# rongzhao-zhang/EfficientQ

Hardware: AMD Instinct MI355X
Metric: ptq_calibration_throughput (higher is better)
Workload: dtype i8xi8->i32 (exact) for the Gram systems and per-iteration loss convs of the layers with quantised input, f32/f64 elsewhere

## Files before the change

efficientq_amd/csrc/solve.hip:

```cpp
#include <cstdlib>
#include <vector>
#include "common.h"
#include "internal.h"

namespace effq {

typedef float f32x16 __attribute__((ext_vector_type(16)));
typedef double f64x4 __attribute__((ext_vector_type(4)));
typedef float f32x4 __attribute__((ext_vector_type(4)));

static inline int round_up(int v, int m) { return (v + m - 1) / m * m; }

constexpr int NBK = 64;
constexpr int LDA_S = 66;
constexpr int LDB_S = 80;

__global__ __launch_bounds__(256) void k_build_a64(const float* __restrict__ A0, int n, int npad, int has_bias,
                                                   double rho, double eta, double* __restrict__ A64) {
  const size_t tot = (size_t)npad * npad;
  const size_t stride = (size_t)gridDim.x * blockDim.x;
  for (size_t e = (size_t)blockIdx.x * blockDim.x + threadIdx.x; e < tot; e += stride) {
    const int i = (int)(e / npad), j = (int)(e % npad);
    double v = 0.0;
    if (i < n && j < n) {
// ... 333 lines not shown
      ra[v] = *reinterpret_cast<const f64x2*>(Ag + v * 32);
      rb[v] = *reinterpret_cast<const f64x2*>(Bg + v * 32);
    }
#pragma unroll
    for (int v = 0; v < 4; ++v) {
      *reinterpret_cast<f64x2*>(&As[0][sk * BG_LD + sc + v * 32]) = ra[v];
      *reinterpret_cast<f64x2*>(&Bs[0][sk * BG_LD + sc + v * 32]) = rb[v];
    }
    lds_barrier();
    for (int c = 0; c < nch; ++c) {
      const int buf = c & 1;
      if (c + 1 < nch) {
        const size_t off = (size_t)(c + 1) * BG_KC * p.ldx;
#pragma unroll
        for (int v = 0; v < 4; ++v) {
          ra[v] = *reinterpret_cast<const f64x2*>(Ag + off + v * 32);
          rb[v] = *reinterpret_cast<const f64x2*>(Bg + off + v * 32);
        }
      }
      if (live) {
#pragma unroll
        for (int ks = 0; ks < BG_KC / 4; ++ks) {
          double a[4], b[4];
#pragma unroll
          for (int mi = 0; mi < 4; ++mi) a[mi] = As[buf][(ks * 4 + lk) * BG_LD + wr * 64 + mi * 16 + lr];
#pragma unroll
          for (int ni = 0; ni < 4; ++ni) b[ni] = Bs[buf][(ks * 4 + lk) * BG_LD + wc * 64 + ni * 16 + lr];
#pragma unroll
          for (int mi = 0; mi < 4; ++mi)
#pragma unroll
            for (int ni = 0; ni < 4; ++ni)
              acc[mi][ni] = __builtin_amdgcn_mfma_f64_16x16x4f64(a[mi], b[ni], acc[mi][ni], 0, 0, 0);
        }
      }
      if (c + 1 < nch) {
#pragma unroll
        for (int v = 0; v < 4; ++v) {
          *reinterpret_cast<f64x2*>(&As[buf ^ 1][sk * BG_LD + sc + v * 32]) = ra[v];
          *reinterpret_cast<f64x2*>(&Bs[buf ^ 1][sk * BG_LD + sc + v * 32]) = rb[v];
        }
      }
      lds_barrier();
    }
  }
  if (live) {
    double* Ob = p.Cout + ((size_t)bi * NBK - p.orow) * p.ldout + ((size_t)bj * NBK - p.ocol);
#pragma unroll
    for (int mi = 0; mi < 4; ++mi)
#pragma unroll
      for (int ni = 0; ni < 4; ++ni)
#pragma unroll
        for (int r = 0; r < 4; ++r) Ob[(size_t)(mi * 16 + lk + 4 * r) * p.ldout + ni * 16 + lr] = acc[mi][ni][r];
  }
}

__global__ __launch_bounds__(256) void k_gj_panel_w(const double* __restrict__ A, int npad, int kb0, int m,
                                                    const double* __restrict__ Dw, double* __restrict__ NZT,
                                                    double* __restrict__ XTW, size_t ldx) {
  extern __shared__ __attribute__((aligned(16))) double sm[];
  double* As = sm;
  double* Bs = sm + NBK * LDA_S;
  const int t = blockIdx.x, c = blockIdx.y;
  if (t >= kb0 && t < kb0 + m) return;
  const int tid = threadIdx.x, lane = tid & 63, wid = tid >> 6;
  const int wr = wid >> 1, wc = wid & 1;
  const bool upper = t < kb0;
  const double sgn = upper ? -1.0 : 1.0;
  const int ldd = m * NBK;
  f64x4 acc[2][2];
#pragma unroll
  for (int mi = 0; mi < 2; ++mi)
#pragma unroll
    for (int ni = 0; ni < 2; ++ni)
#pragma unroll
      for (int r = 0; r < 4; ++r) acc[mi][ni][r] = 0.0;
  for (int a = 0; a < m; ++a) {
    for (int e = tid; e < NBK * NBK; e += 256) {
      const int r = e >> 6, cc = e & 63;
      if (upper)
        As[r * LDA_S + cc] = A[(size_t)(t * NBK + r) * npad + (size_t)(kb0 + a) * NBK + cc];
      else
        As[cc * LDA_S + r] = A[(size_t)((kb0 + a) * NBK + r) * npad + (size_t)t * NBK + cc];
    }
    load_tile(Bs, LDB_S, Dw + (size_t)a * NBK * ldd + (size_t)c * NBK, (size_t)ldd);
    lds_barrier();
    if (a == c)
      for (int e = tid; e < NBK * NBK; e += 256) {
        const int kk = e >> 6, r = e & 63;
        XTW[(size_t)(c * NBK + kk) * ldx + (size_t)t * NBK + r] = sgn * As[r * LDA_S + kk];
      }
    tile_mma64(As, Bs, acc);
    lds_barrier();
  }
  const int lr = lane & 15, lk = lane >> 4;
#pragma unroll
  for (int mi = 0; mi < 2; ++mi)
#pragma unroll
    for (int ni = 0; ni < 2; ++ni)
#pragma unroll
      for (int r = 0; r < 4; ++r)
        As[(wr * 32 + mi * 16 + lk + 4 * r) * LDA_S + wc * 32 + ni * 16 + lr] = acc[mi][ni][r];
  lds_barrier();
  for (int e = tid; e < NBK * NBK; e += 256) {
    const int kk = e >> 6, r = e & 63;
    NZT[(size_t)(c * NBK + kk) * ldx + (size_t)t * NBK + r] = -As[r * LDA_S + kk];
  }
}

__global__ __launch_bounds__(256) void k_gj_wback_w(double* __restrict__ A, int npad, int kb0, int m,
                                                    const double* __restrict__ Dw, const double* __restrict__ NZT,
                                                    size_t ldx) {
  __shared__ double Ts[NBK * (NBK + 1)];
  const int t = blockIdx.x, c = blockIdx.y, tid = threadIdx.x;
  const int ldd = m * NBK;
  if (t >= kb0 && t < kb0 + m) {
    const int a = t - kb0;
    if (a > c) return;
    for (int e = tid; e < NBK * NBK; e += 256) {
      const int r = e >> 6, cc = e & 63;
      A[(size_t)(t * NBK + r) * npad + (size_t)(kb0 + c) * NBK + cc] = Dw[(size_t)(a * NBK + r) * ldd + (size_t)c * NBK + cc];
    }
    return;
  }
  if (t < kb0) {
    for (int e = tid; e < NBK * NBK; e += 256) {
      const int kk = e >> 6, r = e & 63;
      Ts[kk * (NBK + 1) + r] = NZT[(size_t)(c * NBK + kk) * ldx + (size_t)t * NBK + r];
    }
    __syncthreads();
    for (int e = tid; e < NBK * NBK; e += 256) {
      const int r = e >> 6, kk = e & 63;
      A[(size_t)(t * NBK + r) * npad + (size_t)(kb0 + c) * NBK + kk] = Ts[kk * (NBK + 1) + r];
    }
  } else {
    for (int e = tid; e < NBK * NBK; e += 256) {
      const int kk = e >> 6, r = e & 63;
      A[(size_t)((kb0 + c) * NBK + kk) * npad + (size_t)t * NBK + r] = -NZT[(size_t)(c * NBK + kk) * ldx + (size_t)t * NBK + r];
    }
  }
}

constexpr int PF_LD = 130;
__device__ __forceinline__ f64x4 mm16(f64x4 acc, const double* Aop, int a_rs, int a_cs, const double* Bop, int b_rs,
                                      int b_cs, int K, int lr, int lk) {
#pragma unroll 4
  for (int ks = 0; ks < K / 4; ++ks) {
    const double a = Aop[lr * a_rs + (ks * 4 + lk) * a_cs];
    const double b = Bop[(ks * 4 + lk) * b_rs + lr * b_cs];
    acc = __builtin_amdgcn_mfma_f64_16x16x4f64(a, b, acc, 0, 0, 0);
  }
  return acc;
}

__global__ __launch_bounds__(1024) void k_gj_pivot_fused(const double* __restrict__ A, int npad, int k0, int mk,
                                                         const double* __restrict__ NZT, const double* __restrict__ XTW,
                                                         size_t ldx, int kdim, double* __restrict__ Dw) {
  extern __shared__ __attribute__((aligned(16))) double sm[];
  double* M = sm;
  double(*fcol)[NBK + 1] = reinterpret_cast<double(*)[NBK + 1]>(sm + 2 * NBK * PF_LD);
  const int tid = threadIdx.x, lane = tid & 63, wid = tid >> 6;
  const int tr = wid >> 2, tc = wid & 3;
  const int lr = lane & 15, lk = lane >> 4;
  for (int bi = 0; bi < mk; ++bi)
    for (int bj = bi; bj < mk; ++bj) {
      const size_t row0 = (size_t)(k0 + bi) * NBK + tr * 16, col0 = (size_t)(k0 + bj) * NBK + tc * 16;
      f64x4 acc;
#pragma unroll
      for (int r = 0; r < 4; ++r) acc[r] = A[(row0 + lk + 4 * r) * npad + col0 + lr];
      const double* Ag = NZT + row0 + lr;
      const double* Bg = XTW + col0 + lr;
#pragma unroll 8
      for (int ks = 0; ks < kdim / 4; ++ks) {
        const double a = Ag[(size_t)(ks * 4 + lk) * ldx];
        const double b = Bg[(size_t)(ks * 4 + lk) * ldx];
        acc = __builtin_amdgcn_mfma_f64_16x16x4f64(a, b, acc, 0, 0, 0);
      }
#pragma unroll
      for (int r = 0; r < 4; ++r) {
        const int rr = bi * NBK + tr * 16 + lk + 4 * r, cc = bj * NBK + tc * 16 + lr;
        M[rr * PF_LD + cc] = acc[r];
        if (bi < bj) M[cc * PF_LD + rr] = acc[r];
      }
    }
  lds_barrier();
  constexpr int CPW = NBK / 16;
  auto invert64 = [&](int off) {
    double reg[CPW];
#pragma unroll
    for (int j = 0; j < CPW; ++j) reg[j] = M[(off + lane) * PF_LD + off + wid * CPW + j];
    gj_invert_regs<CPW>(reg, fcol, lane, wid);
#pragma unroll
    for (int j = 0; j < CPW; ++j) M[(off + lane) * PF_LD + off + wid * CPW + j] = reg[j];
    lds_barrier();
  };
  auto zero = []() {
    f64x4 z;
#pragma unroll
    for (int r = 0; r < 4; ++r) z[r] = 0.0;
    return z;
  };
  auto tile_store = [&](int rb, int cb, f64x4 v, double sgn) {
#pragma unroll
    for (int r = 0; r < 4; ++r) M[(rb + tr * 16 + lk + 4 * r) * PF_LD + cb + tc * 16 + lr] = sgn * v[r];
  };
  auto tile_load = [&](int rb, int cb) {
    f64x4 v;
#pragma unroll
    for (int r = 0; r < 4; ++r) v[r] = M[(rb + tr * 16 + lk + 4 * r) * PF_LD + cb + tc * 16 + lr];
    return v;
  };
  invert64(0);
  if (mk == 2) {
    f64x4 z = mm16(zero(), M + (NBK + tr * 16) * PF_LD, PF_LD, 1, M + tc * 16, PF_LD, 1, NBK, lr, lk);
    lds_barrier();
    tile_store(NBK, 0, z, 1.0);
    lds_barrier();
    f64x4 sacc = tile_load(NBK, NBK);
#pragma unroll
    for (int r = 0; r < 4; ++r) sacc[r] = -sacc[r];
    sacc = mm16(sacc, M + (NBK + tr * 16) * PF_LD, PF_LD, 1, M + NBK + tc * 16, PF_LD, 1, NBK, lr, lk);
    tile_store(NBK, NBK, sacc, -1.0);
    lds_barrier();
    invert64(NBK);
    f64x4 w = mm16(zero(), M + (NBK + tr * 16) * PF_LD + NBK, PF_LD, 1, M + NBK * PF_LD + tc * 16, PF_LD, 1, NBK, lr, lk);
    tile_store(0, NBK, w, 1.0);
    lds_barrier();
    f64x4 d = tile_load(0, 0);
    d = mm16(d, M + NBK * PF_LD + tr * 16, 1, PF_LD, M + NBK + tc * 16, PF_LD, 1, NBK, lr, lk);
    tile_store(0, 0, d, 1.0);
    lds_barrier();
  }
  const int nd = mk * NBK;
  for (int e = tid; e < nd * nd; e += 1024) {
    const int i = e / nd, j = e % nd;
    double v;
    if (i < NBK && j >= NBK)
      v = -M[(j - NBK) * PF_LD + NBK + i];
    else if (i >= NBK && j < NBK)
      v = -M[(i - NBK) * PF_LD + NBK + j];
    else
      v = M[i * PF_LD + j];
    Dw[e] = v;
  }
}

__global__ __launch_bounds__(256) void k_mirror_blocks(double* __restrict__ D, int nd) {
  const size_t tot = (size_t)nd * nd;
  for (size_t e = (size_t)blockIdx.x * blockDim.x + threadIdx.x; e < tot; e += (size_t)gridDim.x * blockDim.x) {
    const int i = (int)(e / nd), j = (int)(e % nd);
    if ((i / NBK) > (j / NBK)) D[e] = D[(size_t)j * nd + i];
  }
}

__global__ __launch_bounds__(256) void k_build_b(const float* __restrict__ B0, const float* __restrict__ W0,
                                                 const float* __restrict__ b0, const float* __restrict__ G,
                                                 const float* __restrict__ dual, int c2, int n, int has_bias,
                                                 float rho, float eta, float* __restrict__ Bm, int ldb, int c2p,
                                                 const float* __restrict__ wprev, float shift) {
  const size_t tot = (size_t)c2p * ldb;
  const size_t stride = (size_t)gridDim.x * blockDim.x;
  const int nw = n - has_bias;
  for (size_t e = (size_t)blockIdx.x * blockDim.x + threadIdx.x; e < tot; e += stride) {
    const int r = (int)(e / ldb), k = (int)(e % ldb);
    float v = 0.0f;
    if (r < c2 && k < n) {
      if (k < nw) {
        const size_t wi = (size_t)r * nw + k;
        v = B0[(size_t)r * n + k] + eta * W0[wi];
        v = v + rho * (G[wi] - dual[wi]);
        if (wprev != nullptr) v = v + shift * wprev[wi];
      } else {
        v = B0[(size_t)r * n + k] + eta * b0[r];
      }
    }
    Bm[e] = v;
  }
}

__global__ __launch_bounds__(256) void k_build_b4(const float* __restrict__ B0, const float* __restrict__ W0,
                                                  const float* __restrict__ b0, const float* __restrict__ G,
                                                  const float* __restrict__ dual, int c2, int n, int has_bias,
                                                  float rho, float eta, float* __restrict__ Bm, int ldb,
                                                  const float* __restrict__ wprev, float shift) {
  __builtin_amdgcn_s_setprio(2);

  const int r = blockIdx.y;
  const int nw = n - has_bias;
  float* out = Bm + (size_t)r * ldb;
  for (int k = (blockIdx.x * blockDim.x + threadIdx.x) * 4; k < ldb; k += gridDim.x * blockDim.x * 4) {
    float4 v = make_float4(0.f, 0.f, 0.f, 0.f);
    if (r < c2 && k < nw) {
      const size_t wi = (size_t)r * nw + k;
      const float* bp = B0 + (size_t)r * n + k;
      const float4 w0 = *reinterpret_cast<const float4*>(W0 + wi), g = *reinterpret_cast<const float4*>(G + wi),
                   du = *reinterpret_cast<const float4*>(dual + wi);
      v.x = bp[0] + eta * w0.x;
      v.y = bp[1] + eta * w0.y;
      v.z = bp[2] + eta * w0.z;
      v.w = bp[3] + eta * w0.w;
      v.x = v.x + rho * (g.x - du.x);
      v.y = v.y + rho * (g.y - du.y);
      v.z = v.z + rho * (g.z - du.z);
      v.w = v.w + rho * (g.w - du.w);
      if (wprev != nullptr) {
        const float4 wp = *reinterpret_cast<const float4*>(wprev + wi);
        v.x = v.x + shift * wp.x;
        v.y = v.y + shift * wp.y;
        v.z = v.z + shift * wp.z;
        v.w = v.w + shift * wp.w;
      }
    } else if (r < c2 && k == nw && has_bias) {
      v.x = B0[(size_t)r * n + k] + eta * b0[r];
    }
    *reinterpret_cast<float4*>(out + k) = v;
  }
}

__global__ __launch_bounds__(256) void k_prox_reduce4(const float* __restrict__ part, int ldp, int nsplit, int c2, int n,
                                                      int has_bias, float* __restrict__ wstar, float* __restrict__ bstar) {
  __builtin_amdgcn_s_setprio(2);

  const int r = blockIdx.y;
  const int nw = n - has_bias;
  const size_t tot = (size_t)c2 * ldp;
  const float* row = part + (size_t)r * ldp;
  for (int k = (blockIdx.x * blockDim.x + threadIdx.x) * 4; k < ldp; k += gridDim.x * blockDim.x * 4) {
    if (k >= n) continue;
    float4 v = *reinterpret_cast<const float4*>(row + k);
    for (int z = 1; z < nsplit; ++z) {
      const float4 t = *reinterpret_cast<const float4*>(row + (size_t)z * tot + k);
      v.x += t.x;
      v.y += t.y;
      v.z += t.z;
      v.w += t.w;
    }
    if (k < nw)
      *reinterpret_cast<float4*>(wstar + (size_t)r * nw + k) = v;
    else
      bstar[r] = v.x;
  }
}

constexpr int PBK = 32, PLD = PBK + 4;

template <int MT, int WM, int WN, int NTN>
__global__ __launch_bounds__(256) void k_prox_gemm(const float* __restrict__ Bm, int ldb, const float* __restrict__ Ainv,
                                                   int lda, int n, int c2, int has_bias, float* __restrict__ wstar,
                                                   float* __restrict__ bstar, float* __restrict__ part, int ldp) {
  __builtin_amdgcn_s_setprio(2);

  constexpr int BM = 32 * MT * WM, BN = 32 * WN * NTN;
  constexpr int NA = BM * 8 / 256, NB = BN * 8 / 256;
  static_assert(WM * WN == 4 && NA >= 1 && NB >= 1, "4 waves");
  __shared__ __attribute__((aligned(16))) float As[BM * PLD];
  __shared__ __attribute__((aligned(16))) float Bs[BN * PLD];
  const int tid = threadIdx.x, lane = tid & 63, wid = tid >> 6;
  const int li = lane & 31, lh = lane >> 5;
  const int wm = wid / WN, wn = wid % WN;
  const int row0 = blockIdx.y * BM, col0 = blockIdx.x * BN;

  f32x16 acc[MT][NTN];
#pragma unroll
  for (int m = 0; m < MT; ++m)
#pragma unroll
    for (int t = 0; t < NTN; ++t)
#pragma unroll
      for (int r = 0; r < 16; ++r) acc[m][t][r] = 0.0f;

  f32x4 ra[NA], rb[NB];
  const float* pa[NA];
  const float* pb[NB];
#pragma unroll
  for (int q = 0; q < NA; ++q) {
    const int u = tid + q * 256, r = u >> 3, c4 = u & 7;
    pa[q] = Bm + (size_t)(row0 + r) * ldb + c4 * 4;
  }
#pragma unroll
  for (int q = 0; q < NB; ++q) {
    const int u = tid + q * 256, r = u >> 3, c4 = u & 7;
    pb[q] = Ainv + (size_t)min(col0 + r, n - 1) * lda + c4 * 4;
  }
#define EFFQ_PROX_FETCH(k0)                                                         \
  {                                                                                 \
    _Pragma("unroll") for (int q = 0; q < NA; ++q)                                  \
        ra[q] = *reinterpret_cast<const f32x4*>(pa[q] + (k0));                      \
    _Pragma("unroll") for (int q = 0; q < NB; ++q)                                  \
        rb[q] = *reinterpret_cast<const f32x4*>(pb[q] + (k0));                      \
  }
  const int nkt = ldb / PBK;
  const int kt0 = (int)(((long long)nkt * blockIdx.z) / gridDim.z);
  const int nk = (int)(((long long)nkt * (blockIdx.z + 1)) / gridDim.z);
  EFFQ_PROX_FETCH(kt0 * PBK)
  for (int kt = kt0; kt < nk; ++kt) {
    lds_barrier();
#pragma unroll
    for (int q = 0; q < NA; ++q) {
      const int u = tid + q * 256;
      *reinterpret_cast<f32x4*>(&As[(u >> 3) * PLD + (u & 7) * 4]) = ra[q];
    }
#pragma unroll
    for (int q = 0; q < NB; ++q) {
      const int u = tid + q * 256;
      *reinterpret_cast<f32x4*>(&Bs[(u >> 3) * PLD + (u & 7) * 4]) = rb[q];
// ... 112 lines not shown
  }
#define EFFQ_B3_FETCH(k0)                                                           \
  {                                                                                 \
    _Pragma("unroll") for (int q = 0; q < NA; ++q)                                  \
        ra[q] = *reinterpret_cast<const f32x4*>(pa[q] + (k0));                      \
    _Pragma("unroll") for (int q = 0; q < NB; ++q)                                  \
        rb[q] = *reinterpret_cast<const f32x4*>(pb[q] + (k0));                      \
  }
#define EFFQ_B3_STORE(stage)                                                                        \
  {                                                                                                 \
    __bf16* As_ = lds + (stage) * STAGE;                                                            \
    __bf16* Bs_ = As_ + 3 * BM * B3_LD;                                                             \
    _Pragma("unroll") for (int q = 0; q < NA; ++q) {                                                \
      const int u = tid + q * 512, off = (u >> 2) * B3_LD + (u & 3) * 4;                            \
      bf16x4 p0, p1, p2;                                                                            \
      split3(ra[q], p0, p1, p2);                                                                    \
      *reinterpret_cast<bf16x4*>(&As_[off]) = p0;                                                   \
      *reinterpret_cast<bf16x4*>(&As_[BM * B3_LD + off]) = p1;                                      \
      *reinterpret_cast<bf16x4*>(&As_[2 * BM * B3_LD + off]) = p2;                                  \
    }                                                                                               \
    _Pragma("unroll") for (int q = 0; q < NB; ++q) {                                                \
      const int u = tid + q * 512, off = (u >> 2) * B3_LD + (u & 3) * 4;                            \
      bf16x4 p0, p1, p2;                                                                            \
      split3(rb[q], p0, p1, p2);                                                                    \
      *reinterpret_cast<bf16x4*>(&Bs_[off]) = p0;                                                   \
      *reinterpret_cast<bf16x4*>(&Bs_[BN * B3_LD + off]) = p1;                                      \
      *reinterpret_cast<bf16x4*>(&Bs_[2 * BN * B3_LD + off]) = p2;                                  \
    }                                                                                               \
  }
  const int nkt = ldb / B3_K;
  const int kt0 = (int)(((long long)nkt * blockIdx.z) / gridDim.z);
  const int nk = (int)(((long long)nkt * (blockIdx.z + 1)) / gridDim.z);
  EFFQ_B3_FETCH(kt0 * B3_K)
  EFFQ_B3_STORE(0)
  EFFQ_B3_FETCH(min(kt0 + 1, nk - 1) * B3_K)
  lds_barrier();
  for (int kt = kt0; kt < nk; ++kt) {
    const int st = (kt - kt0) & 1;
    if (kt + 1 < nk) EFFQ_B3_STORE(st ^ 1)
    EFFQ_B3_FETCH(min(kt + 2, nk - 1) * B3_K)
    const __bf16* As = lds + st * STAGE;
    const __bf16* Bs = As + 3 * BM * B3_LD;
    bf16x8 a[MT][3], b[NT][3];
#pragma unroll
    for (int m = 0; m < MT; ++m)
#pragma unroll
      for (int p = 0; p < 3; ++p)
        a[m][p] = *reinterpret_cast<const bf16x8*>(&As[p * BM * B3_LD + ((wm * MT + m) * 32 + li) * B3_LD + 8 * lh]);
#pragma unroll
    for (int t = 0; t < NT; ++t)
#pragma unroll
      for (int p = 0; p < 3; ++p)
        b[t][p] = *reinterpret_cast<const bf16x8*>(&Bs[p * BN * B3_LD + ((wn * NT + t) * 32 + li) * B3_LD + 8 * lh]);
#pragma unroll
    for (int m = 0; m < MT; ++m)
#pragma unroll
      for (int t = 0; t < NT; ++t) {
        acc[m][t] = __builtin_amdgcn_mfma_f32_32x32x16_bf16(a[m][0], b[t][2], acc[m][t], 0, 0, 0);
        acc[m][t] = __builtin_amdgcn_mfma_f32_32x32x16_bf16(a[m][1], b[t][1], acc[m][t], 0, 0, 0);
        acc[m][t] = __builtin_amdgcn_mfma_f32_32x32x16_bf16(a[m][2], b[t][0], acc[m][t], 0, 0, 0);
        acc[m][t] = __builtin_amdgcn_mfma_f32_32x32x16_bf16(a[m][0], b[t][1], acc[m][t], 0, 0, 0);
        acc[m][t] = __builtin_amdgcn_mfma_f32_32x32x16_bf16(a[m][1], b[t][0], acc[m][t], 0, 0, 0);
        acc[m][t] = __builtin_amdgcn_mfma_f32_32x32x16_bf16(a[m][0], b[t][0], acc[m][t], 0, 0, 0);
      }
    lds_barrier();
  }
#undef EFFQ_B3_FETCH
#undef EFFQ_B3_STORE
  const int nw = n - has_bias;
  float* P = (gridDim.z > 1) ? part + (size_t)blockIdx.z * c2 * ldp : nullptr;
#pragma unroll
  for (int m = 0; m < MT; ++m)
#pragma unroll
    for (int t = 0; t < NT; ++t) {
      const int col = col0 + (wn * NT + t) * 32 + li;
#pragma unroll
      for (int r = 0; r < 16; ++r) {
        const int row = row0 + (wm * MT + m) * 32 + (r & 3) + 8 * (r >> 2) + 4 * lh;
        if (row < c2 && col < n) {
          if (P != nullptr)
            P[(size_t)row * ldp + col] = acc[m][t][r];
          else if (col < nw)
            wstar[(size_t)row * nw + col] = acc[m][t][r];
          else
            bstar[row] = acc[m][t][r];
        }
      }
    }
}

__global__ __launch_bounds__(256) void k_prox_reduce(const float* __restrict__ part, int ldp, int nsplit, int c2, int n,
                                                     int has_bias, float* __restrict__ wstar, float* __restrict__ bstar) {
  const size_t tot = (size_t)c2 * ldp, stride = (size_t)gridDim.x * blockDim.x;
  const int nw = n - has_bias;
  for (size_t e = (size_t)blockIdx.x * blockDim.x + threadIdx.x; e < tot; e += stride) {
    const int row = (int)(e / ldp), col = (int)(e % ldp);
    if (col >= n) continue;
    float v = part[e];
    for (int z = 1; z < nsplit; ++z) v += part[(size_t)z * tot + e];
    if (col < nw)
      wstar[(size_t)row * nw + col] = v;
    else
      bstar[row] = v;
  }
}

struct ProxPlan { int variant, gx, gy, nsplit, c2p, ldb; };
static ProxPlan prox_plan(int c2, int n) {
  ProxPlan p;
  p.c2p = (c2 > 128) ? round_up(c2, 256) : (c2 > 64) ? 128 : round_up(c2, 32);
  p.ldb = round_up(n, 32);
  if (p.c2p >= 128 && n >= 1024) {
    p.variant = 5; p.gx = (n + 255) / 256; p.gy = p.c2p / 256;
    if (p.c2p == 128) { p.variant = 7; p.gx = (n + 127) / 128; p.gy = 1; }
    const int tiles5 = p.gx * p.gy, nkt5 = p.ldb / B3_K;
    int s5 = (256 + tiles5 / 2) / tiles5;
    if (s5 > nkt5 / 16) s5 = nkt5 / 16;
    if (s5 < 1) s5 = 1;
    p.nsplit = s5;
    return p;
  }
  if (p.c2p >= 256) { p.variant = 0; p.gx = (n + 63) / 64; p.gy = p.c2p / 256; }
  else if (p.c2p == 128) { p.variant = 1; p.gx = (n + 63) / 64; p.gy = 1; }
  else if (p.c2p == 64) { p.variant = 2; p.gx = (n + 63) / 64; p.gy = 1; }
  else { p.variant = 3; p.gx = (n + 127) / 128; p.gy = 1; }
  const int tiles = p.gx * p.gy, nkt = p.ldb / PBK;
  int s = (440 + tiles - 1) / tiles;
  if (s > nkt / 6) s = nkt / 6;
  if (s > 16) s = 16;
  if (s < 1) s = 1;
  if (p.variant == 0) {
    const int smax = s > 1 ? 16 : 1;
    double best = -1.0;
    for (int c = 1; c <= smax && c <= nkt / 6; ++c) {
      const int wgs = tiles * c, rounds = (wgs + 767) / 768;
      const double score = (double)wgs / (768.0 * rounds) - 0.01 * c;
      if (score > best) { best = score; s = c; }
    }
  }
  p.nsplit = s;
  return p;
}

}

using namespace effq;

extern "C" {

static size_t gj64_aux_doubles(size_t npad) { return 2 * (size_t)NBK * npad + 2 * NBK * NBK; }

constexpr int GJ_WIDE_MIN_BLOCKS = 100;
static bool gj_takes_wide(int nblk) { return nblk >= GJ_WIDE_MIN_BLOCKS; }
static int gj_wide_pivot(int nblk) { return (nblk >= 100) ? effq::WB : 2; }

size_t effq_spd_inverse_ws_bytes(int n) {
  if (n <= 0) return 0;
  const size_t npad = (size_t)round_up(n, NBK);
  size_t d = npad * npad + gj64_aux_doubles(npad);
  if (gj_takes_wide((int)(npad / NBK))) {
    const size_t ldx = (size_t)round_up((int)npad, BG_T);
    d = npad * npad + 2 * (size_t)WK * ldx + (size_t)WK * WK + gj64_aux_doubles(WK);
  }
  return d * sizeof(double) + 256;
}

int effq_ainv_ld(int n) { return n > 0 ? round_up(n, 32) : 0; }

static int gj64_sweep(double* A64, int npad, double* aux, hipStream_t st) {
  const int nblk = npad / NBK;
  double* XT = aux;
  double* NZ = XT + (size_t)NBK * npad;
  double* Dinv = NZ + (size_t)NBK * npad;
  const size_t lds = (size_t)(NBK * LDA_S + NBK * LDB_S) * sizeof(double);
  for (int k = 0; k < nblk; ++k) {
    const int kb = k * NBK;
    double* Dk = Dinv + (size_t)(k & 1) * NBK * NBK;
    double* Dn = Dinv + (size_t)((k + 1) & 1) * NBK * NBK;
    if (k == 0) hipLaunchKernelGGL(k_gj_diag, dim3(1), dim3(GJD_T), 0, st, A64, npad, kb, Dk);
    hipLaunchKernelGGL(k_gj_panel, dim3(nblk), dim3(256), lds, st, A64, npad, kb, Dk, NZ, XT);
    if (nblk > 1)
      hipLaunchKernelGGL(k_gj_trail_sym, dim3((nblk + GJ_CT - 1) / GJ_CT, nblk + 1), dim3(256), 0, st, A64, npad, kb, NZ,
                         XT, Dn);
    EFFQ_LAUNCH_CHECK();
  }
  return EFFQ_OK;
}

struct GjWideCtx {
  int dev;
  hipStream_t caller, helper;
  hipEvent_t e1, e2;
};
static thread_local std::vector<GjWideCtx> g_gj_ctx;

static int gj_wide_ctx(hipStream_t caller, GjWideCtx** out) {
  int dev = 0;
  EFFQ_HIP(hipGetDevice(&dev));
  for (GjWideCtx& c : g_gj_ctx)
    if (c.dev == dev && c.caller == caller) {
      *out = &c;
      return EFFQ_OK;
    }
  GjWideCtx c;
  c.dev = dev;
  c.caller = caller;
  int prio = 0;
  if (hipStreamGetPriority(caller, &prio) != hipSuccess) prio = 0;
  EFFQ_HIP(hipStreamCreateWithPriority(&c.helper, hipStreamNonBlocking, prio));
  EFFQ_HIP(hipEventCreateWithFlags(&c.e1, hipEventDisableTiming));
  EFFQ_HIP(hipEventCreateWithFlags(&c.e2, hipEventDisableTiming));
  g_gj_ctx.push_back(c);
  *out = &g_gj_ctx.back();
  return EFFQ_OK;
}

static int gj_wide_sweep(double* A64, int npad, double* aux, hipStream_t st) {
  const int nblk = npad / NBK;
  const int WB = gj_wide_pivot(nblk);
  const size_t ldx = (size_t)round_up(npad, BG_T);
  double* NZT = aux;
  double* XTW = NZT + (size_t)WK * ldx;
  double* Dw = XTW + (size_t)WK * ldx;
  double* aux64 = Dw + (size_t)WK * WK;
  const int nK = (nblk + WB - 1) / WB, nm = (nblk + 1) / 2;
  GjWideCtx* ctx = nullptr;
  if (nK > 1) {
    const int rc = gj_wide_ctx(st, &ctx);
    if (rc != EFFQ_OK) return rc;
  }
  hipStream_t s2 = ctx ? ctx->helper : st;
  const size_t lds = (size_t)(NBK * LDA_S + NBK * LDB_S) * sizeof(double);
  const size_t pf_lds = (size_t)(2 * NBK * PF_LD + 2 * (NBK + 1)) * sizeof(double);
  auto pivot_block = [&](int k0, int mk, int kdim, hipStream_t s) -> int {
    GjBig g;
    memset(&g, 0, sizeof(g));
    g.Cin = A64; g.ldin = (size_t)npad;
    g.Cout = Dw; g.ldout = (size_t)mk * NBK; g.orow = k0 * NBK; g.ocol = k0 * NBK;
    g.NZT = NZT; g.XTW = XTW; g.ldx = ldx; g.kdim = kdim; g.nblk = nblk;
    g.i0m = k0 / 2; g.j0m = k0 / 2;
    g.skip_lo = g.skip_hi = -1; g.la_lo = g.la_hi = -1;
    if (WB == 2) {
      hipLaunchKernelGGL(k_gj_pivot_fused, dim3(1), dim3(1024), pf_lds, s, A64, npad, k0, mk, NZT, XTW, ldx, kdim, Dw);
      EFFQ_LAUNCH_CHECK();
      return EFFQ_OK;
    }
    const int span = (mk + 1) / 2;
    hipLaunchKernelGGL(k_gj_big, dim3(span, span), dim3(256), 0, s, g);
    EFFQ_LAUNCH_CHECK();
    const int rc = gj64_sweep(Dw, mk * NBK, aux64, s);
    if (rc != EFFQ_OK) return rc;
    hipLaunchKernelGGL(k_mirror_blocks, dim3(64), dim3(256), 0, s, Dw, mk * NBK);
    EFFQ_LAUNCH_CHECK();
    return EFFQ_OK;
  };
  {
    const int rc = pivot_block(0, nblk < WB ? nblk : WB, 0, st);
    if (rc != EFFQ_OK) return rc;
  }
  for (int K = 0; K < nK; ++K) {
    const int kb0 = K * WB, m = (nblk - kb0 < WB) ? nblk - kb0 : WB;
    const int kn0 = kb0 + WB, mn = (K + 1 < nK) ? ((nblk - kn0 < WB) ? nblk - kn0 : WB) : 0;
    hipLaunchKernelGGL(k_gj_panel_w, dim3(nblk, m), dim3(256), lds, st, A64, npad, kb0, m, Dw, NZT, XTW, ldx);
    EFFQ_LAUNCH_CHECK();
    if (ctx) {
      EFFQ_HIP(hipEventRecord(ctx->e1, st));
      EFFQ_HIP(hipStreamWaitEvent(s2, ctx->e1, 0));
    }
    hipLaunchKernelGGL(k_gj_wback_w, dim3(nblk, m), dim3(256), 0, s2, A64, npad, kb0, m, Dw, NZT, ldx);
    EFFQ_LAUNCH_CHECK();
    if (mn > 0) {
      const int rc = pivot_block(kn0, mn, m * NBK, s2);
      if (rc != EFFQ_OK) return rc;
    }
    if (nblk > m) {
      GjBig g;
      memset(&g, 0, sizeof(g));
      g.Cin = A64; g.ldin = (size_t)npad;
      g.Cout = A64; g.ldout = (size_t)npad; g.orow = 0; g.ocol = 0;
      g.NZT = NZT; g.XTW = XTW; g.ldx = ldx; g.kdim = m * NBK; g.nblk = nblk;
      g.i0m = 0; g.j0m = 0;
      g.skip_lo = kb0; g.skip_hi = kb0 + m;
      g.la_lo = mn > 0 ? kn0 : -1; g.la_hi = mn > 0 ? kn0 + mn : -1;
      hipLaunchKernelGGL(k_gj_big, dim3(nm, nm), dim3(256), 0, st, g);
      EFFQ_LAUNCH_CHECK();
    }
    if (ctx) {
      EFFQ_HIP(hipEventRecord(ctx->e2, s2));
      EFFQ_HIP(hipStreamWaitEvent(st, ctx->e2, 0));
    }
  }
  return EFFQ_OK;
}

int effq_spd_inverse_prepare(void* stream) {
  GjWideCtx* ctx = nullptr;
  return gj_wide_ctx(as_stream(stream), &ctx);
}

int effq_spd_inverse(const float* A0, int n, int has_bias, double rho, double eta, float* Ainv, void* ws,
                     size_t ws_bytes, void* stream) {
  EFFQ_CHECK_ARG(A0 && Ainv && ws && n > 0);
  EFFQ_CHECK_ARG(eta > 0.0 && rho >= 0.0);
  if (ws_bytes < effq_spd_inverse_ws_bytes(n)) {
    set_error("spd_inverse: workspace %zu < required %zu", ws_bytes, effq_spd_inverse_ws_bytes(n));
    return EFFQ_ERR_WORKSPACE;
  }
  const int npad = round_up(n, NBK);
  double* A64 = reinterpret_cast<double*>(ws);
  double* aux = A64 + (size_t)npad * npad;
  hipStream_t st = as_stream(stream);
  {
    size_t nb = ((size_t)npad * npad + 255) / 256;
    if (nb > 8192) nb = 8192;
    hipLaunchKernelGGL(k_build_a64, dim3((unsigned)nb), dim3(256), 0, st, A0, n, npad, has_bias, rho, eta, A64);
    EFFQ_LAUNCH_CHECK();
  }
  const size_t lds = (size_t)(NBK * LDA_S + NBK * LDB_S) * sizeof(double);
  EFFQ_HIP(raise_lds_limit<k_gj_panel>(lds));
  EFFQ_HIP(raise_lds_limit<k_gj_panel_w>(lds));
  EFFQ_HIP(raise_lds_limit<k_gj_pivot_fused>((2 * NBK * PF_LD + 2 * (NBK + 1)) * sizeof(double)));
  const int rc = gj_takes_wide(npad / NBK) ? gj_wide_sweep(A64, npad, aux, st) : gj64_sweep(A64, npad, aux, st);
  if (rc != EFFQ_OK) return rc;
  {
    const int lda = effq_ainv_ld(n);
    size_t nb = ((size_t)n * lda + 255) / 256;
    if (nb > 8192) nb = 8192;
    hipLaunchKernelGGL(k_a64_to_f32, dim3((unsigned)nb), dim3(256), 0, st, A64, n, npad, Ainv, lda);
    EFFQ_LAUNCH_CHECK();
  }
  return EFFQ_OK;
}

int effq_spd_inverse_plan(int n, int* wide, int* nblk, int* pivot_blocks) {
  EFFQ_CHECK_ARG(n > 0 && wide && nblk && pivot_blocks);
  const int nb = round_up(n, NBK) / NBK;
  *wide = gj_takes_wide(nb) ? 1 : 0;
  *nblk = nb;
  *pivot_blocks = *wide ? (nb + gj_wide_pivot(nb) - 1) / gj_wide_pivot(nb) : nb;
  return EFFQ_OK;
}

int effq_prox_plan_query(int c2, int n, int* variant, int* gx, int* gy, int* nsplit) {
  EFFQ_CHECK_ARG(c2 > 0 && n > 0 && variant && gx && gy && nsplit);
  const ProxPlan p = prox_plan(c2, n);
  *variant = p.variant;
  *gx = p.gx;
  *gy = p.gy;
  *nsplit = p.nsplit;
  return EFFQ_OK;
}

size_t effq_prox_ws_bytes(int c2, int n) {
  if (c2 <= 0 || n <= 0) return 0;
  const ProxPlan p = prox_plan(c2, n);
  return ((size_t)p.c2p + (p.nsplit > 1 ? (size_t)p.nsplit * c2 : 0)) * p.ldb * sizeof(float) + 256;
}

static int prox_solve_impl(const float* B0, const float* Ainv, const float* W0, const float* b0, const float* G,
                           const float* dual, int c2, int n, int has_bias, double rho, double eta, double shift,
                           int nterms, float* wstar, float* bstar, void* ws, size_t ws_bytes, void* stream,
                           bool prebuilt = false, const float** part_out = nullptr, int* nsplit_out = nullptr,
                           int* ldp_out = nullptr) {
  EFFQ_CHECK_ARG(B0 && Ainv && W0 && G && dual && wstar && ws && c2 > 0 && n > 0 && nterms >= 1);
  EFFQ_CHECK_ARG(!has_bias || (b0 != nullptr && bstar != nullptr));
  if (ws_bytes < effq_prox_ws_bytes(c2, n)) {
    set_error("prox_solve: workspace %zu < required %zu", ws_bytes, effq_prox_ws_bytes(c2, n));
    return EFFQ_ERR_WORKSPACE;
  }
  const ProxPlan pl = prox_plan(c2, n);
  const int c2p = pl.c2p, ldb = pl.ldb;
  const int lda = effq_ainv_ld(n);
  float* Bm = reinterpret_cast<float*>(ws);
  float* part = Bm + (size_t)c2p * ldb;
  hipStream_t st = as_stream(stream);
  for (int term = 0; term < nterms; ++term) {
    if (!(prebuilt && term == 0)) {
      const int nw = n - (has_bias ? 1 : 0);
      if ((nw % 4) == 0) {
        const unsigned bx = (unsigned)((ldb / 4 + 255) / 256);
        hipLaunchKernelGGL(k_build_b4, dim3(bx, (unsigned)c2p), dim3(256), 0, st, B0, W0, b0, G, dual, c2, n,
                           has_bias ? 1 : 0, (float)rho, (float)eta, Bm, ldb, (term > 0) ? wstar : nullptr, (float)shift);
      } else {
        size_t nb = ((size_t)c2p * ldb + 255) / 256;
        if (nb > 4096) nb = 4096;
        hipLaunchKernelGGL(k_build_b, dim3((unsigned)nb), dim3(256), 0, st, B0, W0, b0, G, dual, c2, n, has_bias ? 1 : 0,
                           (float)rho, (float)eta, Bm, ldb, c2p, (term > 0) ? wstar : nullptr, (float)shift);
      }
      EFFQ_LAUNCH_CHECK();
    }
    const dim3 grid(pl.gx, pl.gy, pl.nsplit);
#define EFFQ_PROX_LAUNCH(MT, WM, WN, NTN)                                                                              \
  hipLaunchKernelGGL((k_prox_gemm<MT, WM, WN, NTN>), grid, dim3(256), 0, st, Bm, ldb, Ainv, lda, n, c2, has_bias ? 1 : 0, \
                     wstar, bstar, part, ldb)
    if (pl.variant == 5 || pl.variant == 7) {
      const size_t lds5 = (size_t)2 * 3 * (256 + 256) * B3_LD * sizeof(__bf16);
      const size_t lds7 = (size_t)2 * 3 * (128 + 128) * B3_LD * sizeof(__bf16);
      EFFQ_HIP((raise_lds_limit<k_prox_gemm_b3<256, 256, 4, 2>>(lds5)));
      EFFQ_HIP((raise_lds_limit<k_prox_gemm_b3<128, 128, 2, 4>>(lds7)));
      if (pl.variant == 5)
        hipLaunchKernelGGL((k_prox_gemm_b3<256, 256, 4, 2>), grid, dim3(512), lds5, st, Bm, ldb, Ainv, lda, n, c2,
                           has_bias ? 1 : 0, wstar, bstar, part, ldb);
      else
        hipLaunchKernelGGL((k_prox_gemm_b3<128, 128, 2, 4>), grid, dim3(512), lds7, st, Bm, ldb, Ainv, lda, n, c2,
                           has_bias ? 1 : 0, wstar, bstar, part, ldb);
    } else
    switch (pl.variant) {
      case 0: EFFQ_PROX_LAUNCH(2, 4, 1, 2); break;
      case 1: EFFQ_PROX_LAUNCH(1, 4, 1, 2); break;
      case 2: EFFQ_PROX_LAUNCH(1, 2, 2, 1); break;
      default: EFFQ_PROX_LAUNCH(1, 1, 4, 1); break;
    }
#undef EFFQ_PROX_LAUNCH
    EFFQ_LAUNCH_CHECK();
    if (part_out != nullptr) {
      *part_out = (pl.nsplit > 1) ? part : nullptr;
      *nsplit_out = pl.nsplit;
      *ldp_out = ldb;
    } else if (pl.nsplit > 1) {
      const int nw = n - (has_bias ? 1 : 0);
      if ((nw % 4) == 0) {
        const unsigned bx = (unsigned)((ldb / 4 + 255) / 256);
        hipLaunchKernelGGL(k_prox_reduce4, dim3(bx, (unsigned)c2), dim3(256), 0, st, part, ldb, pl.nsplit, c2, n,
                           has_bias ? 1 : 0, wstar, bstar);
      } else {
        size_t nb = ((size_t)c2 * ldb + 255) / 256;
        if (nb > 2048) nb = 2048;
        hipLaunchKernelGGL(k_prox_reduce, dim3((unsigned)nb), dim3(256), 0, st, part, ldb, pl.nsplit, c2, n,
                           has_bias ? 1 : 0, wstar, bstar);
      }
      EFFQ_LAUNCH_CHECK();
    }
  }
  return EFFQ_OK;
}

int effq_prox_solve(const float* B0, const float* Ainv, const float* W0, const float* b0, const float* G,
                    const float* dual, int c2, int n, int has_bias, double rho, double eta, float* wstar, float* bstar,
                    void* ws, size_t ws_bytes, void* stream) {
  return prox_solve_impl(B0, Ainv, W0, b0, G, dual, c2, n, has_bias, rho, eta, 0.0, 1, wstar, bstar, ws, ws_bytes,
                         stream);
}

float* effq_prox_bm(void* ws, int c2, int n, int* ldb) {
  *ldb = prox_plan(c2, n).ldb;
  return reinterpret_cast<float*>(ws);
}
int effq_prox_solve_prebuilt(const float* B0, const float* Ainv, const float* W0, const float* b0, const float* G,
                             const float* dual, int c2, int n, int has_bias, double rho, double eta, float* wstar,
                             float* bstar, void* ws, size_t ws_bytes, void* stream) {
  return prox_solve_impl(B0, Ainv, W0, b0, G, dual, c2, n, has_bias, rho, eta, 0.0, 1, wstar, bstar, ws, ws_bytes,
                         stream, true);
}

int effq_prox_solve_prebuilt_parts(const float* B0, const float* Ainv, const float* W0, const float* b0, const float* G,
                                   const float* dual, int c2, int n, int has_bias, double rho, double eta, float* wstar,
                                   float* bstar, void* ws, size_t ws_bytes, void* stream, const float** part_out,
                                   int* nsplit_out, int* ldp_out) {
  EFFQ_CHECK_ARG(part_out && nsplit_out && ldp_out);
  return prox_solve_impl(B0, Ainv, W0, b0, G, dual, c2, n, has_bias, rho, eta, 0.0, 1, wstar, bstar, ws, ws_bytes,
                         stream, true, part_out, nsplit_out, ldp_out);
}

int effq_prox_solve_shifted(const float* B0, const float* Ainv, const float* W0, const float* b0, const float* G,
                            const float* dual, int c2, int n, int has_bias, double rho, double eta, double rho_inv,
                            int nterms, float* wstar, float* bstar, void* ws, size_t ws_bytes, void* stream) {
  EFFQ_CHECK_ARG(rho_inv >= rho && rho > 0.0 && eta >= 0.0);
  return prox_solve_impl(B0, Ainv, W0, b0, G, dual, c2, n, has_bias, rho, eta, rho_inv - rho, nterms, wstar, bstar, ws,
                         ws_bytes, stream);
}

}
```

Baseline: 24.88.

## Invert wide GJ pivot blocks with fused two-stage kernels and double-buffered pivot workspace

The wide Gauss-Jordan sweep previously inverted each WB-block pivot by running a full gj64 sweep (many small launches) followed by a mirror kernel. Now it applies a Schur-complement scheme: a fused single-workgroup kernel inverts the leading 2x2 block and forms the coupling panel, and a second fused launch inverts the Schur complement and updates the remaining blocks. The pivot kernel writes the full symmetric result directly, so the mirror pass is gone. The pivot inverse is double-buffered so that the next pivot can be computed on the helper stream before the current write-back, which adds workspace and ordering complexity.

```diff
diff --git a/efficientq_amd/csrc/solve.hip b/efficientq_amd/csrc/solve.hip
--- a/efficientq_amd/csrc/solve.hip
+++ b/efficientq_amd/csrc/solve.hip
@@ -509,27 +509,45 @@
   return acc;
 }
 
-__global__ __launch_bounds__(1024) void k_gj_pivot_fused(const double* __restrict__ A, int npad, int k0, int mk,
-                                                         const double* __restrict__ NZT, const double* __restrict__ XTW,
-                                                         size_t ldx, int kdim, double* __restrict__ Dw) {
+struct GjPivot {
+  const double* A;
+  size_t lda;
+  int mk;
+  const double* NZr;
+  const double* XTc;
+  size_t ldx;
+  int kdim;
+  double* Out;
+  size_t ldo;
+  int tail;
+  const double* T01;
+  size_t ldt;
+  double* NZ2;
+  size_t ldn;
+  int nc;
+  double* O;
+};
+
+__global__ __launch_bounds__(1024) void k_gj_pivot_fused(const GjPivot p) {
   extern __shared__ __attribute__((aligned(16))) double sm[];
   double* M = sm;
   double(*fcol)[NBK + 1] = reinterpret_cast<double(*)[NBK + 1]>(sm + 2 * NBK * PF_LD);
   const int tid = threadIdx.x, lane = tid & 63, wid = tid >> 6;
   const int tr = wid >> 2, tc = wid & 3;
   const int lr = lane & 15, lk = lane >> 4;
+  const int mk = p.mk;
   for (int bi = 0; bi < mk; ++bi)
     for (int bj = bi; bj < mk; ++bj) {
-      const size_t row0 = (size_t)(k0 + bi) * NBK + tr * 16, col0 = (size_t)(k0 + bj) * NBK + tc * 16;
+      const size_t row0 = (size_t)bi * NBK + tr * 16, col0 = (size_t)bj * NBK + tc * 16;
       f64x4 acc;
 #pragma unroll
-      for (int r = 0; r < 4; ++r) acc[r] = A[(row0 + lk + 4 * r) * npad + col0 + lr];
-      const double* Ag = NZT + row0 + lr;
-      const double* Bg = XTW + col0 + lr;
+      for (int r = 0; r < 4; ++r) acc[r] = p.A[(row0 + lk + 4 * r) * p.lda + col0 + lr];
+      const double* Ag = p.NZr + row0 + lr;
+      const double* Bg = p.XTc + col0 + lr;
 #pragma unroll 8
-      for (int ks = 0; ks < kdim / 4; ++ks) {
-        const double a = Ag[(size_t)(ks * 4 + lk) * ldx];
-        const double b = Bg[(size_t)(ks * 4 + lk) * ldx];
+      for (int ks = 0; ks < p.kdim / 4; ++ks) {
+        const double a = Ag[(size_t)(ks * 4 + lk) * p.ldx];
+        const double b = Bg[(size_t)(ks * 4 + lk) * p.ldx];
         acc = __builtin_amdgcn_mfma_f64_16x16x4f64(a, b, acc, 0, 0, 0);
       }
 #pragma unroll
@@ -586,26 +604,61 @@
     d = mm16(d, M + NBK * PF_LD + tr * 16, 1, PF_LD, M + NBK + tc * 16, PF_LD, 1, NBK, lr, lk);
     tile_store(0, 0, d, 1.0);
     lds_barrier();
+    for (int e = tid; e < NBK * NBK; e += 1024) {
+      const int i = e >> 6, j = e & 63;
+      M[(NBK + i) * PF_LD + j] = -M[i * PF_LD + NBK + j];
+    }
+    lds_barrier();
+    for (int e = tid; e < NBK * NBK; e += 1024) {
+      const int i = e >> 6, j = e & 63;
+      M[i * PF_LD + NBK + j] = M[(NBK + j) * PF_LD + i];
+    }
+    lds_barrier();
   }
   const int nd = mk * NBK;
   for (int e = tid; e < nd * nd; e += 1024) {
     const int i = e / nd, j = e % nd;
-    double v;
-    if (i < NBK && j >= NBK)
-      v = -M[(j - NBK) * PF_LD + NBK + i];
-    else if (i >= NBK && j < NBK)
-      v = -M[(i - NBK) * PF_LD + NBK + j];
-    else
-      v = M[i * PF_LD + j];
-    Dw[e] = v;
-  }
-}
-
-__global__ __launch_bounds__(256) void k_mirror_blocks(double* __restrict__ D, int nd) {
-  const size_t tot = (size_t)nd * nd;
-  for (size_t e = (size_t)blockIdx.x * blockDim.x + threadIdx.x; e < tot; e += (size_t)gridDim.x * blockDim.x) {
-    const int i = (int)(e / nd), j = (int)(e % nd);
-    if ((i / NBK) > (j / NBK)) D[e] = D[(size_t)j * nd + i];
+    p.Out[(size_t)i * p.ldo + j] = M[i * PF_LD + j];
+  }
+  if (p.tail == 1) {
+    for (int a = 0; a < 2; ++a)
+      for (int b = 0; b < p.nc / NBK; ++b) {
+        const int ti = tr + 4 * a, tj = tc + 4 * b;
+        f64x4 v = zero();
+        for (int h = 0; h < 2 * NBK; h += NBK)
+          v = mm16(v, M + ti * 16 * PF_LD + h, PF_LD, 1, p.T01 + h * p.ldt + tj * 16, (int)p.ldt, 1, NBK, lr, lk);
+#pragma unroll
+        for (int r = 0; r < 4; ++r) p.NZ2[(size_t)(ti * 16 + lk + 4 * r) * p.ldn + tj * 16 + lr] = -v[r];
+      }
+  } else if (p.tail == 2) {
+    for (int a = 0; a < 2; ++a)
+      for (int b = 0; b < p.nc / NBK; ++b) {
+        const int ti = tr + 4 * a, tj = tc + 4 * b;
+        f64x4 v = zero();
+        for (int h = 0; h < p.nc; h += NBK)
+          v = mm16(v, p.NZ2 + (size_t)ti * 16 * p.ldn + h, (int)p.ldn, 1, M + h * PF_LD + tj * 16, PF_LD, 1, NBK, lr, lk);
+#pragma unroll
+        for (int r = 0; r < 4; ++r) {
+          const size_t i = ti * 16 + lk + 4 * r, c = 2 * NBK + tj * 16 + lr;
+          p.O[i * p.ldo + c] = v[r];
+          p.O[c * p.ldo + i] = v[r];
+        }
+      }
+    __threadfence_block();
+    __syncthreads();
+    for (int a = 0; a < 2; ++a)
+      for (int b = 0; b < 2; ++b) {
+        const int ti = tr + 4 * a, tj = tc + 4 * b;
+        double* Ot = p.O + (size_t)ti * 16 * p.ldo + tj * 16;
+        f64x4 v;
+#pragma unroll
+        for (int r = 0; r < 4; ++r) v[r] = Ot[(size_t)(lk + 4 * r) * p.ldo + lr];
+        for (int h = 0; h < p.nc; h += NBK)
+          v = mm16(v, p.NZ2 + (size_t)ti * 16 * p.ldn + h, (int)p.ldn, 1, p.O + (size_t)tj * 16 * p.ldo + 2 * NBK + h, 1,
+                   (int)p.ldo, NBK, lr, lk);
+#pragma unroll
+        for (int r = 0; r < 4; ++r) Ot[(size_t)(lk + 4 * r) * p.ldo + lr] = v[r];
+      }
   }
 }
 
@@ -1024,16 +1077,16 @@
 
 constexpr int GJ_WIDE_MIN_BLOCKS = 100;
 static bool gj_takes_wide(int nblk) { return nblk >= GJ_WIDE_MIN_BLOCKS; }
-static int gj_wide_pivot(int nblk) { return (nblk >= 100) ? effq::WB : 2; }
+
+static size_t gj_wide_aux_doubles(size_t npad) {
+  const size_t ldx = (size_t)round_up((int)npad, BG_T);
+  return 2 * (size_t)WK * ldx + 2 * (size_t)WK * WK + 2 * (size_t)NBK * WK;
+}
 
 size_t effq_spd_inverse_ws_bytes(int n) {
   if (n <= 0) return 0;
   const size_t npad = (size_t)round_up(n, NBK);
-  size_t d = npad * npad + gj64_aux_doubles(npad);
-  if (gj_takes_wide((int)(npad / NBK))) {
-    const size_t ldx = (size_t)round_up((int)npad, BG_T);
-    d = npad * npad + 2 * (size_t)WK * ldx + (size_t)WK * WK + gj64_aux_doubles(WK);
-  }
+  const size_t d = npad * npad + (gj_takes_wide((int)(npad / NBK)) ? gj_wide_aux_doubles(npad) : gj64_aux_doubles(npad));
   return d * sizeof(double) + 256;
 }
 
@@ -1089,12 +1142,11 @@
 
 static int gj_wide_sweep(double* A64, int npad, double* aux, hipStream_t st) {
   const int nblk = npad / NBK;
-  const int WB = gj_wide_pivot(nblk);
   const size_t ldx = (size_t)round_up(npad, BG_T);
   double* NZT = aux;
   double* XTW = NZT + (size_t)WK * ldx;
-  double* Dw = XTW + (size_t)WK * ldx;
-  double* aux64 = Dw + (size_t)WK * WK;
+  double* Dw2 = XTW + (size_t)WK * ldx;
+  double* NZ2 = Dw2 + 2 * (size_t)WK * WK;
   const int nK = (nblk + WB - 1) / WB, nm = (nblk + 1) / 2;
   GjWideCtx* ctx = nullptr;
   if (nK > 1) {
@@ -1104,47 +1156,61 @@
   hipStream_t s2 = ctx ? ctx->helper : st;
   const size_t lds = (size_t)(NBK * LDA_S + NBK * LDB_S) * sizeof(double);
   const size_t pf_lds = (size_t)(2 * NBK * PF_LD + 2 * (NBK + 1)) * sizeof(double);
-  auto pivot_block = [&](int k0, int mk, int kdim, hipStream_t s) -> int {
+  auto pivot_block = [&](int k0, int mk, int kdim, double* Dw, hipStream_t s) -> int {
+    const size_t ldd = (size_t)mk * NBK;
+    GjPivot q;
+    memset(&q, 0, sizeof(q));
+    if (mk <= 2) {
+      q.A = A64 + (size_t)k0 * NBK * npad + (size_t)k0 * NBK; q.lda = (size_t)npad; q.mk = mk;
+      q.NZr = NZT + (size_t)k0 * NBK; q.XTc = XTW + (size_t)k0 * NBK; q.ldx = ldx; q.kdim = kdim;
+      q.Out = Dw; q.ldo = ldd;
+      hipLaunchKernelGGL(k_gj_pivot_fused, dim3(1), dim3(1024), pf_lds, s, q);
+      EFFQ_LAUNCH_CHECK();
+      return EFFQ_OK;
+    }
     GjBig g;
     memset(&g, 0, sizeof(g));
     g.Cin = A64; g.ldin = (size_t)npad;
-    g.Cout = Dw; g.ldout = (size_t)mk * NBK; g.orow = k0 * NBK; g.ocol = k0 * NBK;
+    g.Cout = Dw; g.ldout = ldd; g.orow = k0 * NBK; g.ocol = k0 * NBK;
     g.NZT = NZT; g.XTW = XTW; g.ldx = ldx; g.kdim = kdim; g.nblk = nblk;
     g.i0m = k0 / 2; g.j0m = k0 / 2;
     g.skip_lo = g.skip_hi = -1; g.la_lo = g.la_hi = -1;
-    if (WB == 2) {
-      hipLaunchKernelGGL(k_gj_pivot_fused, dim3(1), dim3(1024), pf_lds, s, A64, npad, k0, mk, NZT, XTW, ldx, kdim, Dw);
-      EFFQ_LAUNCH_CHECK();
-      return EFFQ_OK;
-    }
     const int span = (mk + 1) / 2;
     hipLaunchKernelGGL(k_gj_big, dim3(span, span), dim3(256), 0, s, g);
     EFFQ_LAUNCH_CHECK();
-    const int rc = gj64_sweep(Dw, mk * NBK, aux64, s);
-    if (rc != EFFQ_OK) return rc;
-    hipLaunchKernelGGL(k_mirror_blocks, dim3(64), dim3(256), 0, s, Dw, mk * NBK);
+    q.A = Dw; q.lda = ldd; q.mk = 2; q.kdim = 0; q.NZr = NZ2; q.XTc = NZ2; q.ldx = ldd;
+    q.Out = Dw; q.ldo = ldd;
+    q.tail = 1; q.T01 = Dw + 2 * NBK; q.ldt = ldd; q.NZ2 = NZ2; q.ldn = ldd; q.nc = (mk - 2) * NBK; q.O = Dw;
+    hipLaunchKernelGGL(k_gj_pivot_fused, dim3(1), dim3(1024), pf_lds, s, q);
+    EFFQ_LAUNCH_CHECK();
+    q.A = Dw + (size_t)2 * NBK * ldd + 2 * NBK; q.mk = mk - 2; q.kdim = 2 * NBK; q.XTc = Dw + 2 * NBK;
+    q.Out = Dw + (size_t)2 * NBK * ldd + 2 * NBK;
+    q.tail = 2;
+    hipLaunchKernelGGL(k_gj_pivot_fused, dim3(1), dim3(1024), pf_lds, s, q);
     EFFQ_LAUNCH_CHECK();
     return EFFQ_OK;
   };
   {
-    const int rc = pivot_block(0, nblk < WB ? nblk : WB, 0, st);
+    const int rc = pivot_block(0, nblk < WB ? nblk : WB, 0, Dw2, st);
     if (rc != EFFQ_OK) return rc;
   }
   for (int K = 0; K < nK; ++K) {
     const int kb0 = K * WB, m = (nblk - kb0 < WB) ? nblk - kb0 : WB;
     const int kn0 = kb0 + WB, mn = (K + 1 < nK) ? ((nblk - kn0 < WB) ? nblk - kn0 : WB) : 0;
+    double* Dw = Dw2 + (size_t)(K & 1) * WK * WK;
+    double* Dn = Dw2 + (size_t)((K + 1) & 1) * WK * WK;
     hipLaunchKernelGGL(k_gj_panel_w, dim3(nblk, m), dim3(256), lds, st, A64, npad, kb0, m, Dw, NZT, XTW, ldx);
     EFFQ_LAUNCH_CHECK();
     if (ctx) {
       EFFQ_HIP(hipEventRecord(ctx->e1, st));
       EFFQ_HIP(hipStreamWaitEvent(s2, ctx->e1, 0));
     }
+    if (mn > 0) {
+      const int rc = pivot_block(kn0, mn, m * NBK, Dn, s2);
+      if (rc != EFFQ_OK) return rc;
+    }
     hipLaunchKernelGGL(k_gj_wback_w, dim3(nblk, m), dim3(256), 0, s2, A64, npad, kb0, m, Dw, NZT, ldx);
     EFFQ_LAUNCH_CHECK();
-    if (mn > 0) {
-      const int rc = pivot_block(kn0, mn, m * NBK, s2);
-      if (rc != EFFQ_OK) return rc;
-    }
     if (nblk > m) {
       GjBig g;
       memset(&g, 0, sizeof(g));
@@ -1209,7 +1275,7 @@
   const int nb = round_up(n, NBK) / NBK;
   *wide = gj_takes_wide(nb) ? 1 : 0;
   *nblk = nb;
-  *pivot_blocks = *wide ? (nb + gj_wide_pivot(nb) - 1) / gj_wide_pivot(nb) : nb;
+  *pivot_blocks = *wide ? (nb + WB - 1) / WB : nb;
   return EFFQ_OK;
 }
 
```

Result: slower. 24.59 (-1.2%).
